# metaverse3d2022/Nerf-Cuda

Hardware: AMD Instinct MI355X
Metric: megasamples/s (march samples composited into a ray = the reference's per-ray sample count), Lego-like NeRF render @1920x1080 (higher is better)
Workload: dtype f16

## Files before the change

### nerf-cuda_amd/csrc/nrf_device.h

```cpp
#pragma once

#include <hip/hip_runtime.h>
#include <stdint.h>

#include "../../include/nerfhip.h"

namespace nrf {

typedef _Float16 half_t;
typedef _Float16 half2_t __attribute__((ext_vector_type(2)));
typedef _Float16 half4_t __attribute__((ext_vector_type(4)));
typedef _Float16 half8_t __attribute__((ext_vector_type(8)));
typedef float float2_t __attribute__((ext_vector_type(2)));
typedef float float4_t __attribute__((ext_vector_type(4)));

enum : uint32_t {
  LV_DENSE = 0,
  LV_HASH_POW2 = 1,
  LV_GENERIC = 2,
  LV_ADD_POW2 = 3
};

struct LevelParams {
  float scale;
// ... 610 lines not shown
  const uint32_t row = __umul24(gy, L.q_my_b) + L.q_off_b;
  const uint32_t slab = __umul24(gz, L.q_mz_b) + row;
  const uint32_t off0 = (gx << 4) + slab;
  const uint32_t off1 = off0 + L.q_mz_b;
  const __amdgpu_buffer_rsrc_t rsrc = __builtin_amdgcn_make_buffer_rsrc(const_cast<uint32_t*>(grid), 0, grid_bytes, 0x00020000);
  typedef uint32_t u32x4 __attribute__((ext_vector_type(4)));
  const u32x4 a = __builtin_amdgcn_raw_buffer_load_b128(rsrc, off0, 0, 0);
  const u32x4 b = __builtin_amdgcn_raw_buffer_load_b128(rsrc, off1, 0, 0);
  v[0] = a.x; v[1] = a.y; v[2] = a.z; v[3] = a.w;
  v[4] = b.x; v[5] = b.y; v[6] = b.z; v[7] = b.w;
}

__device__ __forceinline__ void level_gather_quad_far(const uint32_t* __restrict__ grid, const LevelParams L, float px, float py, float pz,
                                                      uint32_t (&v)[8], float (&frac)[3]) {
  float fx = px * L.scale; fx = fx + 0.5f;
  float fy = py * L.scale; fy = fy + 0.5f;
  float fz = pz * L.scale; fz = fz + 0.5f;
  uint32_t gx = (uint32_t)(int)fx, gy = (uint32_t)(int)fy, gz = (uint32_t)(int)fz;
  frac[0] = __builtin_amdgcn_fractf(fx);
  frac[1] = __builtin_amdgcn_fractf(fy);
  frac[2] = __builtin_amdgcn_fractf(fz);
  gx = gx < L.q_max ? gx : L.q_max;
  gy = gy < L.q_max ? gy : L.q_max;
  gz = gz < L.q_max ? gz : L.q_max;
  const uint32_t row = __umul24(gy, L.q_my_b) + L.q_off_b;
  const uint32_t cell = __umul24(gz, L.q_mz_b) + row + gx;
  const uint4* q = reinterpret_cast<const uint4*>(grid) + cell;
  const uint4 a = q[0];
  const uint4 b = q[L.q_mz_b];
  v[0] = a.x; v[1] = a.y; v[2] = a.z; v[3] = a.w;
  v[4] = b.x; v[5] = b.y; v[6] = b.z; v[7] = b.w;
}

template <bool FAST = false>
__device__ __forceinline__ uint32_t level_interp(const uint32_t (&v)[8], const float (&frac)[3]) {
  const float wx[2] = {1 - frac[0], frac[0]};
  const float wy[2] = {1 - frac[1], frac[1]};
  const float wz[2] = {1 - frac[2], frac[2]};
  if constexpr (FAST) {
    uint32_t a = 0u;
#pragma unroll
    for (int c = 0; c < 8; ++c) {
      const float w = (wx[c & 1] * wy[(c >> 1) & 1]) * wz[(c >> 2) & 1];
      asm("v_fma_mixlo_f16 %0, %1, %2, %0 op_sel_hi:[0,1,1]" : "+v"(a) : "v"(w), "v"(v[c]));
      asm("v_fma_mixhi_f16 %0, %1, %2, %0 op_sel:[0,1,1] op_sel_hi:[0,1,1]" : "+v"(a) : "v"(w), "v"(v[c]));
    }
    return a;
  }
  half2_t acc = {(half_t)0.0f, (half_t)0.0f};
#ifdef NRF_DIAG_DROP_INTERP_CVT
  float diag_acc_lo = 0.f, diag_acc_hi = 0.f;
#endif
#pragma unroll
  for (int c = 0; c < 8; ++c) {
    const float w = (wx[c & 1] * wy[(c >> 1) & 1]) * wz[(c >> 2) & 1];
#ifdef NRF_DIAG_DROP_INTERP_CVT
    {
      float lo, hi;
      const float neg_zero = -0.0f;
      asm("v_fma_mix_f32 %0, %1, %2, %3 op_sel_hi:[0,1,0]" : "=v"(lo) : "v"(w), "v"(v[c]), "v"(neg_zero));
      asm("v_fma_mix_f32 %0, %1, %2, %3 op_sel:[0,1,0] op_sel_hi:[0,1,0]" : "=v"(hi) : "v"(w), "v"(v[c]), "v"(neg_zero));
      diag_acc_lo += lo;
      diag_acc_hi += hi;
    }
#else
    acc = acc + weight_times_entry(w, v[c]);
// ... 201 lines not shown

__device__ __forceinline__ half8_t frag_load(const uint4* wl, int f, int lane) {
  const uint4 v = wl[f * 64 + lane];
  return __builtin_bit_cast(half8_t, v);
}

__device__ __forceinline__ half8_t pack_acc(float4_t lo, float4_t hi) {
#ifdef NRF_PROBE_NO_PACK
  typedef uint32_t u4 __attribute__((ext_vector_type(4)));
  return __builtin_bit_cast(half8_t, __builtin_bit_cast(u4, lo) ^ __builtin_bit_cast(u4, hi));
#endif
  half8_t r;
  r[0] = (half_t)lo[0]; r[1] = (half_t)lo[1]; r[2] = (half_t)lo[2]; r[3] = (half_t)lo[3];
  r[4] = (half_t)hi[0]; r[5] = (half_t)hi[1]; r[6] = (half_t)hi[2]; r[7] = (half_t)hi[3];
  const half8_t zero8 = {(half_t)0.f, (half_t)0.f, (half_t)0.f, (half_t)0.f, (half_t)0.f, (half_t)0.f, (half_t)0.f, (half_t)0.f};
  return __builtin_elementwise_max(r, zero8);
}

struct LdsFrags {
  const uint4* wl;
  int lane;
  __device__ __forceinline__ half8_t operator()(int f) const { return frag_load(wl, f >= FRAG_R0X ? f - FRAG_R0X + N_FRAGS : f, lane); }
};
struct LdsFragsPlain {
  const uint4* wl;
  int lane;
  __device__ __forceinline__ half8_t operator()(int f) const { return frag_load(wl, f, lane); }
};
template <int NT>
struct MlpOut {
  uint32_t rg[NT], bx[NT];
  half_t sigma;
};
template <int NT, int D0_BASE = FRAG_D0, typename Frags = LdsFrags, int RK = 1, int W = 64>
__device__ __forceinline__ void mlp_tiles(const Frags frag, const half8_t (&feat)[NT], const half4_t (&dirf)[NT], MlpOut<NT>& out,
                                          bool rgb_sigmoid = false, const half8_t (*dirx)[RK_WIDE - 1] = nullptr) {
  static_assert(NT == 1 || NT == 2 || NT == 4, "tiles per pass");
  using S = MlpShape<W>;
  constexpr int MT = S::MT, KS = S::KS;
  const float4_t zero = {0.f, 0.f, 0.f, 0.f};
  float4_t acc[NT][MT];
  half8_t hb[NT][KS];
  auto repack = [&]() {
#pragma unroll
    for (int n = 0; n < NT; ++n)
#pragma unroll
      for (int s = 0; s < KS; ++s) hb[n][s] = pack_acc(acc[n][2 * s], 2 * s + 1 < MT ? acc[n][2 * s + 1] : zero);
  };
#pragma unroll
  for (int m = 0; m < MT; ++m) {
    const half8_t a = frag(D0_BASE + m);
#pragma unroll
    for (int n = 0; n < NT; ++n) acc[n][m] = mfma16(a, feat[n], zero);
  }
  repack();
  float4_t dacc[NT];
#pragma unroll
  for (int n = 0; n < NT; ++n) dacc[n] = zero;
#pragma unroll
  for (int s = 0; s < KS; ++s) {
    const half8_t a = frag(S::D1 + s);
#pragma unroll
    for (int n = 0; n < NT; ++n) dacc[n] = mfma16(a, hb[n][s], dacc[n]);
  }
  half8_t rin[NT];
  uint32_t d01[NT];
#pragma unroll
  for (int n = 0; n < NT; ++n) {
    half8_t r;
    r[0] = (half_t)dacc[n][0];
    r[1] = (half_t)dacc[n][1];
    r[2] = (half_t)dacc[n][2];
// ... 185 lines not shown
```

### nerf-cuda_amd/csrc/nrf_launch.h

```cpp
#pragma once
#include <hip/hip_runtime.h>
#include <math.h>
#include <stdint.h>

namespace nrf {
enum : int { NET_HOT = 0, NET_GENERIC = 1, NET_WIDE = 2, NET_W16 = 3, NET_W32 = 4, NET_W128 = 5, NET_WIDE_SH = 6, NET_DEPTH = 7,
             NET_GRID2 = 8, NET_GRID4 = 9, NET_GRID8 = 10, NET_GRID1 = 11, NET_ACT = 12 };
__host__ __device__ constexpr int net_grid_f(int net) {
  return net == NET_GRID2 ? 2 : (net == NET_GRID4 ? 4 : (net == NET_GRID8 ? 8 : (net == NET_GRID1 ? 1 : 0)));
}
__host__ __device__ constexpr int net_width(int net) { return net == NET_W16 ? 16 : (net == NET_W32 ? 32 : (net == NET_W128 ? 128 : 64)); }

enum : uint32_t { GFORM_MIXED = 0, GFORM_DENSE = 1, GFORM_HASHED = 2, GFORM_QUAD = 3, GFORM_QUAD_FAR = 4 };
__host__ __device__ constexpr uint32_t gather_plan(uint32_t f0, uint32_t f1, uint32_t f2, uint32_t f3) {
  return 0x10000u | f0 | (f1 << 4) | (f2 << 8) | (f3 << 12);
}
__host__ __device__ constexpr uint32_t gather_form(uint32_t plan, int jl) { return (plan >> (4 * jl)) & 15u; }
constexpr uint32_t GATHER_RUNTIME = 0;
constexpr uint32_t GATHER_QQFH = gather_plan(GFORM_QUAD, GFORM_QUAD, GFORM_QUAD_FAR, GFORM_HASHED);
constexpr uint32_t GATHER_QQHH = gather_plan(GFORM_QUAD, GFORM_QUAD, GFORM_HASHED, GFORM_HASHED);
constexpr uint32_t GATHER_DMHH = gather_plan(GFORM_DENSE, GFORM_MIXED, GFORM_HASHED, GFORM_HASHED);
inline uint32_t gather_plan_of(int own, uint32_t n_levels, uint32_t uni_modes, uint32_t quad_mask, uint32_t quad_far) {
  if (own != NET_HOT || n_levels != 16) return GATHER_RUNTIME;
  uint32_t f[4];
  for (int jl = 0; jl < 4; ++jl)
    f[jl] = ((quad_mask >> (4 * jl)) & 1u) ? (((quad_far >> jl) & 1u) ? GFORM_QUAD_FAR : GFORM_QUAD) : ((uni_modes >> (2 * jl)) & 3u);
  const uint32_t plan = gather_plan(f[0], f[1], f[2], f[3]);
  return plan == GATHER_QQFH || plan == GATHER_QQHH || plan == GATHER_DMHH ? plan : GATHER_RUNTIME;
}

struct DevModel;
struct FrameParams;
struct ViewBatch;

constexpr int RENDER_QUEUE_BYTES = 8 * 4;
constexpr int WIDE_GENERIC_MARCH_WAVES = 8;
hipError_t launch_render(const DevModel& M, const FrameParams& P, const ViewBatch& VB, void* rgba, void* depth, void* counters,
                         hipStream_t st, bool first_launch, unsigned* plan = nullptr, unsigned plan_cap = 0);
constexpr unsigned PLAN_CAP = 60u * 1024u;
constexpr size_t PLAN_BYTES = (4 + 2 * (size_t)PLAN_CAP) * 4;
hipError_t launch_build_quads(const void* table, uint32_t res, uint32_t size, bool hashed, void* quads, hipStream_t st);
hipError_t launch_encode_grid(const DevModel& M, const void* pos01, uint32_t n, void* out, hipStream_t st, bool fast_interp = false);
hipError_t launch_encode_dir(const DevModel& M, const void* dir01, uint32_t n, void* out, hipStream_t st);
hipError_t launch_mlp_forward(const DevModel& M, const void* feat, const void* dirfeat, uint32_t n, void* out, uint32_t repeat,
                              hipStream_t st);
hipError_t launch_network(const DevModel& M, const void* xyz, const void* dir, uint32_t n, void* sigma, void* rgb, hipStream_t st);
hipError_t launch_density_positions(uint32_t H, float k, void* xyz, void* dir, hipStream_t st);
hipError_t launch_density_update(const void* sigma, uint32_t n, float decay, int n_iterations, void* grid, hipStream_t st);
hipError_t launch_generate_rays(const DevModel& M, const FrameParams& P, void* rays_o, void* rays_d, void* nears, void* fars,
                                hipStream_t st);
hipError_t launch_march(const DevModel& M, float dt_gamma, const void* rays_o, const void* rays_d, const void* rays_t,
                        const void* fars, uint32_t n, uint32_t n_step, void* xyzs, void* dirs, void* deltas, hipStream_t st,
                        uint32_t perturb = 0);
hipError_t launch_composite(const void* sigmas, const void* rgbs, const void* deltas, uint32_t n, uint32_t n_step, void* rays_t,
                            void* state, hipStream_t st);
hipError_t launch_untile(const void* gathered, int shard_count, int tiles_per_shard, int C, int W, int H, int n_views, void* out,
                         hipStream_t st);
hipError_t launch_untile_rgbd8_u8(const void* gathered, int shard_count, int tiles_per_shard, int W, int H, int n_views, void* rgb8,
                                  void* depth8, hipStream_t st);
hipError_t launch_quantize_rgbd8(const void* rgba, const void* depth, uint64_t n, void* out, hipStream_t st);
hipError_t launch_quantize(const void* rgba, const void* depth, int n, void* rgb8, void* depth8, hipStream_t st);
enum : int { MARCH_FORM_GENERIC = 0, MARCH_FORM_UNIT = 1, MARCH_FORM_POW2 = 2 };
inline int march_form(uint32_t H, uint32_t cascade, float bound) {
  const bool pow2_h = H != 0 && (H & (H - 1)) == 0;
  int eb = 0;
  if (pow2_h && cascade == 1 && bound >= 1.0f) return MARCH_FORM_UNIT;
  if (pow2_h && cascade > 1 && bound >= 1.0f && frexpf(bound, &eb) == 0.5f) return MARCH_FORM_POW2;
  return MARCH_FORM_GENERIC;
}
int render_persist_waves(int net, int form);
int render_persistent_lds_bytes(int net, int waves, uint32_t gen_wave_bytes);
void preload_kernels(bool all);
int render_lds_table_max_bytes();
int render_wide_lds_fixed_bytes();
int render_gen_lds_fixed_bytes(uint32_t gen_wave_bytes);
}
```

### nerf-cuda_amd/csrc/nrf_render.h

```cpp

#pragma once
#include <cstddef>
#include <cstdlib>

#include "nrf_device.h"
#include "nrf_generic.h"
#include "nrf_launch.h"

namespace nrf {

#ifndef NRF_SLOTS
#define NRF_SLOTS 64
#endif
constexpr int SLOTS = NRF_SLOTS;
struct WaveLds {
  union {
    float4 pos[SLOTS];
    float4 out[SLOTS];
  };
  float2 aux[SLOTS];
  uint32_t dirf[64][8];
};
static_assert(sizeof(WaveLds) == 2048 + 24 * SLOTS, "WaveLds layout");

// ... 138 lines not shown
          for (int e = 0; e < DW; ++e) fb[DW * jl + e] = o[e];
        }
      }
    }
  }
}

template <int RK, bool SHROWS>
__device__ __forceinline__ void gather_step(const DevModel& M, const LevelParams* lvs, int jl, int g, float px, float py, float pz,
                                            uint32_t (&v)[8], float (&fr)[3]) {
  const LevelParams L = lvs[4 * jl + g];
  const uint32_t uni = (M.uni_modes >> (2 * jl)) & 3u;
  if ((M.quad_mask >> (4 * jl)) & 1u) {
    constexpr bool FARQ = !(RK > 1 && !SHROWS);
    if (FARQ && ((M.quad_far >> jl) & 1u)) level_gather_quad_far(M.grid, L, px, py, pz, v, fr);
    else level_gather_quad(M.grid, M.grid_bytes, L, px, py, pz, v, fr);
  }
  else if (uni == 2u) level_gather<2>(M.grid, M.grid_bytes, L, px, py, pz, v, fr);
  else if (uni == 1u) level_gather<1>(M.grid, M.grid_bytes, L, px, py, pz, v, fr);
  else level_gather<0>(M.grid, M.grid_bytes, L, px, py, pz, v, fr);
}
template <uint32_t GP, int JL>
__device__ __forceinline__ void gather_step_static(const DevModel& M, const LevelParams* lvs, int g, float px, float py, float pz,
                                                   uint32_t (&v)[8], float (&fr)[3]) {
  constexpr uint32_t form = gather_form(GP, JL);
  static_assert(form <= GFORM_QUAD_FAR, "a static gather plan names one of the five step forms");
  const LevelParams L = lvs[4 * JL + g];
  if constexpr (form == GFORM_QUAD_FAR) level_gather_quad_far(M.grid, L, px, py, pz, v, fr);
  else if constexpr (form == GFORM_QUAD) level_gather_quad(M.grid, M.grid_bytes, L, px, py, pz, v, fr);
  else if constexpr (form == GFORM_HASHED) level_gather<2>(M.grid, M.grid_bytes, L, px, py, pz, v, fr);
  else if constexpr (form == GFORM_DENSE) level_gather<1>(M.grid, M.grid_bytes, L, px, py, pz, v, fr);
  else level_gather<0>(M.grid, M.grid_bytes, L, px, py, pz, v, fr);
}
__device__ __forceinline__ void sample_pos01(const DevModel& M, const float4 p, float& px, float& py, float& pz) {
  if (M.pos_w_pow2) {
    px = __builtin_fmaf(M.pos_w, p.x, 0.5f);
    py = __builtin_fmaf(M.pos_w, p.y, 0.5f);
    pz = __builtin_fmaf(M.pos_w, p.z, 0.5f);
  } else {
    px = M.pos_w * p.x; px = px + 0.5f;
    py = M.pos_w * p.y; py = py + 0.5f;
    pz = M.pos_w * p.z; pz = pz + 0.5f;
  }
}

template <int NT, int RK = 1, bool FAST = false, int WD = 64, bool SHROWS = false, int DEPTH = 0, int GF = 0, uint32_t GP = GATHER_RUNTIME>
__device__ __forceinline__ void network_from_lds(const DevModel& M, const uint4* wl, const LevelParams* lvs, WaveLds* W,
                                                 const float* rayd, int S, int base, int lane, float density_scale,
                                                 const half_t* rows = nullptr) {
  const int g = lane >> 4, c = lane & 15;
  half8_t feat[NT];
  half4_t dirf[NT];
  half8_t dirx[NT][RK_WIDE - 1];
#pragma unroll
  for (int n = 0; n < NT; ++n) {
    const int slot = base + 16 * n + c;
    uint32_t fb[4] = {0u, 0u, 0u, 0u};
    uint2 db = make_uint2(0u, 0u);
    if (slot < S) {
      const float4 p = W->pos[slot];
      float px, py, pz;
      sample_pos01(M, p, px, py, pz);
      if constexpr (GF != 0) {
        grid_features<GF>(M, lvs, px, py, pz, g, fb);
      } else {
      uint32_t gv[4][8];
      float gf[4][3];
      if constexpr (GP != GATHER_RUNTIME) {
        static_assert(RK == 1, "static gather plans exist for the hot instance only");
        gather_step_static<GP, 0>(M, lvs, g, px, py, pz, gv[0], gf[0]);
        gather_step_static<GP, 1>(M, lvs, g, px, py, pz, gv[1], gf[1]);
        gather_step_static<GP, 2>(M, lvs, g, px, py, pz, gv[2], gf[2]);
        gather_step_static<GP, 3>(M, lvs, g, px, py, pz, gv[3], gf[3]);
      } else {
#pragma unroll
      for (int jl = 0; jl < 4; ++jl) gather_step<RK, SHROWS>(M, lvs, jl, g, px, py, pz, gv[jl], gf[jl]);
      }
#pragma unroll
      for (int jl = 0; jl < 4; ++jl) fb[jl] = level_interp<FAST>(gv[jl], gf[jl]);
      }
      const int ray = __builtin_bit_cast(int, p.w);
      db = *reinterpret_cast<const uint2*>(&W->dirf[ray][2 * g]);
      if constexpr (RK > 1 && SHROWS) {
        const half8_t z8 = {(half_t)0.f, (half_t)0.f, (half_t)0.f, (half_t)0.f, (half_t)0.f, (half_t)0.f, (half_t)0.f, (half_t)0.f};
#pragma unroll
        for (int s = 1; s < RK; ++s) {
          const uint32_t e0 = 32u * s - 16u + 8u * (uint32_t)g;
          dirx[n][s - 1] = e0 < M.dir_w ? *reinterpret_cast<const half8_t*>(rows + (size_t)ray * SH_ROW_HALVES + e0) : z8;
        }
      } else if constexpr (RK > 1) {
        const float dx = rayd[3 * ray], dy = rayd[3 * ray + 1], dz = rayd[3 * ray + 2];
#pragma unroll
        for (int s = 1; s < RK; ++s) dirx[n][s - 1] = dir_entries8(M.n_frequencies, 32u * s - 16u + 8u * (uint32_t)g, dx, dy, dz);
      }
    } else if constexpr (RK > 1) {
      const half8_t z8 = {(half_t)0.f, (half_t)0.f, (half_t)0.f, (half_t)0.f, (half_t)0.f, (half_t)0.f, (half_t)0.f, (half_t)0.f};
#pragma unroll
      for (int s = 1; s < RK; ++s) dirx[n][s - 1] = z8;
    }
    const uint4 fv = make_uint4(fb[0], fb[1], fb[2], fb[3]);
    feat[n] = __builtin_bit_cast(half8_t, fv);
    dirf[n] = __builtin_bit_cast(half4_t, db);
  }
  MlpOut<NT> o;
  if constexpr (DEPTH == 2) mlp_tiles_depth<NT, LdsFragsPlain, true>(LdsFragsPlain{wl, lane}, feat, dirf, o, M.rgb_output_activation == NRF_ACT_SIGMOID, M.depth_xd,
                                                                     M.depth_xr, M.density_activation, M.rgb_activation);
  else if constexpr (DEPTH == 1) mlp_tiles_depth<NT>(LdsFragsPlain{wl, lane}, feat, dirf, o, M.rgb_output_activation == NRF_ACT_SIGMOID, M.depth_xd, M.depth_xr);
  else if constexpr (WD == 64) mlp_tiles<NT, FRAG_D0, LdsFrags, RK>(LdsFrags{wl, lane}, feat, dirf, o, M.rgb_output_activation == NRF_ACT_SIGMOID, dirx);
  else mlp_tiles<NT, 0, LdsFragsPlain, 1, WD>(LdsFragsPlain{wl, lane}, feat, dirf, o, M.rgb_output_activation == NRF_ACT_SIGMOID);
  if (g == 0) {
#pragma unroll
    for (int n = 0; n < NT; ++n) {
      const int slot = base + 16 * n + c;
      const half2_t rg = bits_h2(o.rg[n]), bx = bits_h2(o.bx[n]);
      if (slot < S) *reinterpret_cast<float3*>(&W->out[slot]) = make_float3((float)rg.x, (float)rg.y, (float)bx.x);
    }
  }
  if (g < NT) {
    const int slot = base + 16 * g + c;
    float sigma = (float)o.sigma;
    if (density_scale != 1.0f) sigma = density_scale * sigma;
    if (slot < S) W->out[slot].w = sigma;
  }
}

constexpr int NT_MAX = 2;

template <bool DENSITY_ONLY>
__device__ __forceinline__ void gen_network_from_lds(const DevModel& M, const GenModel& G, const LevelParams* lvs, WaveLds* W,
                                                     const GenLds& Lw, int S, int base, int lane, float density_scale) {
  const int g = lane >> 4, c = lane & 15;
  float p01[GEN_TILES][3];
  bool valid[GEN_TILES];
  int ray[GEN_TILES];
#pragma unroll
  for (int n = 0; n < GEN_TILES; ++n) {
    const int slot = base + 16 * n + c;
    valid[n] = slot < S;
    ray[n] = 0;
    p01[n][0] = p01[n][1] = p01[n][2] = 0.5f;
// ... 1 lines not shown
      const float4 p = W->pos[slot];
      float px = M.pos_w * p.x; px = px + 0.5f;
      float py = M.pos_w * p.y; py = py + 0.5f;
      float pz = M.pos_w * p.z; pz = pz + 0.5f;
      p01[n][0] = px; p01[n][1] = py; p01[n][2] = pz;
      ray[n] = __builtin_bit_cast(int, p.w) & 63;
    }
  }
  gen_encode_rows(M, G, lvs, Lw, lane, p01, valid);
  if constexpr (!DENSITY_ONLY) {
    const int slot = base + lane;
    if (lane < GEN_SAMPLES && slot < S) {
      const int r = __builtin_bit_cast(int, W->pos[slot].w) & 63;
      gen_encode_dir(M, G, Lw.rayd[3 * r], Lw.rayd[3 * r + 1], Lw.rayd[3 * r + 2], Lw.dir + (size_t)lane * G.dir_stride);
    }
#pragma unroll
    for (int n = 0; n < GEN_TILES; ++n) ray[n] = 16 * n + c;
  }
  gen_wave_sync();
  float4_t o[GEN_TILES];
  gen_mlps<DENSITY_ONLY>(M, G, Lw, lane, ray, o);
  if (g == 0) {
#pragma unroll
    for (int n = 0; n < GEN_TILES; ++n) {
      const int slot = base + 16 * n + c;
      float sigma = o[n][3];
      if (density_scale != 1.0f) sigma = density_scale * sigma;
      if (slot < S) W->out[slot] = make_float4(o[n][0], o[n][1], o[n][2], sigma);
    }
  }
  gen_wave_sync();
}

template <int NET, bool FAST = false, uint32_t GP = GATHER_RUNTIME>
__device__ __forceinline__ void network_dispatch(const DevModel& M, const uint4* wl, const LevelParams* lvs, WaveLds* W,
                                                 const GenLds& Lw, int S, int lane, float density_scale) {
  constexpr int RK = (NET == NET_WIDE || NET == NET_WIDE_SH) ? RK_WIDE : 1;
  constexpr bool SHR = NET == NET_WIDE_SH;
  if constexpr (NET == NET_GENERIC) {
    const GenModel& G = *M.gen;
    for (int base = 0; base < S; base += GEN_SAMPLES)
      gen_network_from_lds<false>(M, G, lvs, W, Lw, S, base, lane, density_scale);
  } else {
    constexpr int WD = net_width(NET);
    constexpr int NTM = WD == 128 ? 1 : NT_MAX;
    for (int base = 0; base < S; base += 16 * NTM) {
      const int ntile = (S - base + 15) >> 4;
      constexpr int DP = NET == NET_DEPTH ? 1 : (NET == NET_ACT ? 2 : 0);
      constexpr int GF = net_grid_f(NET);
      if (ntile <= 1 || NTM == 1) network_from_lds<1, RK, FAST, WD, SHR, DP, GF, GP>(M, wl, lvs, W, Lw.rayd, S, base, lane, density_scale, Lw.dir);
      else network_from_lds<NTM, RK, FAST, WD, SHR, DP, GF, GP>(M, wl, lvs, W, Lw.rayd, S, base, lane, density_scale, Lw.dir);
    }
  }
}

struct LdsMap {
  uint4* wl;
  LevelParams* lvs;
  WaveLds* W;
  GenLds gen;
  unsigned char* tables;
};
template <int NET>
__device__ __forceinline__ LdsMap lds_map(unsigned char* smem, const DevModel& M, int wave, int n_waves) {
  LdsMap m;
  if constexpr (NET == NET_GENERIC) {
    const GenModel& G = *M.gen;
    m.lvs = reinterpret_cast<LevelParams*>(smem);
    unsigned char* waves = smem + LDS_LEVEL_BYTES;
    m.W = reinterpret_cast<WaveLds*>(waves) + wave;
    unsigned char* dir = waves + n_waves * (int)sizeof(WaveLds);
    unsigned char* act = dir + n_waves * gen_dir_bytes(G);
    m.wl = reinterpret_cast<uint4*>(act);
    m.gen.dens = reinterpret_cast<half_t*>(&m.W->dirf[0][0]);
    m.gen.rayd = reinterpret_cast<float*>(&m.W->dirf[32][0]);
    m.gen.dir = reinterpret_cast<half_t*>(dir + wave * gen_dir_bytes(G));
    m.gen.X = reinterpret_cast<half_t*>(act + wave * gen_act_bytes(G));
    m.gen.Y = m.gen.X + GEN_SAMPLES * G.act_stride;
    m.gen.wfrag = M.wfrag;
    m.tables = act + n_waves * gen_act_bytes(G);
  } else {
    constexpr int WF = net_wfrag_bytes(NET);
    m.wl = reinterpret_cast<uint4*>(smem);
    m.lvs = reinterpret_cast<LevelParams*>(smem + WF);
// ... 293 lines not shown
                                                     rdy, rdz, sx, sy, sz, far_m, t_skip, budget, t, x, y, z, dt);
        found = r == MARCH_FOUND;
        marching = found;
        ended = ended || r == MARCH_EXHAUSTED;
      }
#ifdef NRF_PHASE_TIMING
      {
        int used = budget_before - budget;
        n_lane_trips += (unsigned)used;
        for (int o = 32; o; o >>= 1) used = max(used, __shfl_xor(used, o));
        n_wave_iters += (unsigned)used;
      }
#endif
      const unsigned long long fm = __ballot(found);
      if (found) {
        const int slot = S + (int)__builtin_amdgcn_mbcnt_hi((unsigned)(fm >> 32), __builtin_amdgcn_mbcnt_lo((unsigned)fm, 0u));
        const float tn = t + dt;
        const float delta = tn - last_t;
        tc = tc + delta;
        t = tc;
        W->pos[slot] = make_float4(x, y, z, __builtin_bit_cast(float, lane));
        W->aux[slot] = make_float2(dt, tc);
        slots |= (unsigned long long)slot << (8 * k);
        cnt++;
        if (n_ray_samples + cnt >= P.max_steps) { marching = false; ended = true; }
        else if (cnt >= cap) marching = false;
      }
      S += __popcll(fm);
    }
    wave_sync();
    NRF_STAMP(t1);

    if (S > 0) {
      network_dispatch<NET, FAST, GP>(M, wl, lvs, W, lm.gen, S, lane, P.density_scale);
      wave_sync();
    }
    NRF_STAMP(t2);

    if (alive) {
      bool terminated = false;
      for (int k = 0; k < 8; ++k) {
        if (k >= cnt) break;
        const int slot = (int)((slots >> (8 * k)) & 0xffull);
        const float4 so = W->out[slot];
        const float2 dtc = W->aux[slot];
        const float alpha = 1.0f - __expf(-so.w * dtc.x);
        const float T = 1 - ws;
        const float wgt = alpha * T;
        ws += wgt;
        dep += wgt * dtc.y;
        cr += wgt * so.x;
        cg += wgt * so.y;
        cb += wgt * so.z;
        n_comp++;
        if (T <= 9.99999974737875e-05f) { terminated = true; break; }
      }
      n_ray_samples += cnt;
      alive = !(terminated || ended);
    }
    wave_sync();
    NRF_STAMP(t3);
    NRF_ACC(c_march, t0, t1);
    NRF_ACC(c_net, t1, t2);
    NRF_ACC(c_comp, t2, t3);
    n_samples += (unsigned)S;
    n_rounds++;
    n_tile_slots += (unsigned)((S + 15) & ~15);
// ... 303 lines not shown
          uint32_t GP = GATHER_RUNTIME, bool FAST = false>
__global__ __launch_bounds__(64 * WAVES, 1) void render_persistent_kernel(const DevModel M0, const FrameParams P0, const ViewBatch VB0,
                                                                              float4* __restrict__ rgba0, float* __restrict__ depth0,
                                                                              unsigned long long* __restrict__ counters,
                                                                              unsigned* __restrict__ queue) {
  extern __shared__ __attribute__((aligned(16))) unsigned char smem[];
  const int wave = __builtin_amdgcn_readfirstlane((int)(threadIdx.x >> 6));
  const int lane = lane_id();
  typedef const PersistArgs __attribute__((address_space(4))) * KArgPtr;
  KArgPtr ka = (KArgPtr)__builtin_amdgcn_kernarg_segment_ptr();
  const DevModel& M = M0;
  const FrameParams& P = P0;
  const ViewBatch& VB = VB0;
  constexpr int PERSIST_WAVES = WAVES;
  constexpr bool GEN = NET == NET_GENERIC;
  constexpr int OUT8 = U8 ? 1 : 0;
  LdsMap lm = lds_map<NET>(smem, M, wave, PERSIST_WAVES);
  uint32_t* coarse_lds = reinterpret_cast<uint32_t*>(lm.tables);
  float* ctab_lds = reinterpret_cast<float*>(coarse_lds + M.lds_coarse_words);
  uint32_t* dil_lds = reinterpret_cast<uint32_t*>(ctab_lds + M.lds_ctab_floats);
  int* q_lds = reinterpret_cast<int*>(dil_lds + M.lds_dilated_words);
  unsigned* sched = reinterpret_cast<unsigned*>(q_lds + MAX_VIEWS + 1);
  HelpLds* hl = reinterpret_cast<HelpLds*>(sched + 1);
  static_assert(WAVES <= 16, "HelpLds::mail / idle_mask hold 16 waves");
  if constexpr (!GEN) stage_fragments<NET>(M, lm.wl);
  if constexpr (GEN && WLDS) {
    uint4* w_lds = reinterpret_cast<uint4*>(smem + ((reinterpret_cast<unsigned char*>(hl + 1) + LDS_CLOCK_BYTES - smem + 15) & ~(size_t)15));
    for (uint32_t i = threadIdx.x; i < M.gen_frag_bytes / 16u; i += blockDim.x) w_lds[i] = M.wfrag[i];
    lm.gen.wfrag = w_lds;
  }
  for (uint32_t i = threadIdx.x; i < M.lds_coarse_words; i += blockDim.x) coarse_lds[i] = M.occ_coarse[i];
  for (uint32_t i = threadIdx.x; i < M.lds_ctab_floats; i += blockDim.x) ctab_lds[i] = M.cell_bound[i];
  for (uint32_t i = threadIdx.x; i < M.lds_dilated_words; i += blockDim.x) dil_lds[i] = M.occ_dilated[i];
  if (threadIdx.x < 16) lm.lvs[threadIdx.x] = M.lv[threadIdx.x];
  if (threadIdx.x <= MAX_VIEWS) {
    const int v = (int)threadIdx.x;
    q_lds[v] = v < VB.n_views ? VB.v[v].q_begin : VB.q_total;
  }
  if (threadIdx.x == 0) *sched = (0xfffffeu << 5) | 4u;
  if (threadIdx.x == 0) {
    hl->idle_mask = 0u;
    hl->busy = PERSIST_WAVES;
  }
  if (threadIdx.x < 16) hl->mail[threadIdx.x] = 0u;
  __syncthreads();
#ifndef NRF_PHASE_TIMING
  unsigned* clk_lds = reinterpret_cast<unsigned*>(hl + 1);
  if (wave == 0) {
    unsigned long long t0, r0;
    asm volatile("s_memtime %0\n\ts_memrealtime %1\n\ts_waitcnt lgkmcnt(0)" : "=s"(t0), "=s"(r0)::"memory");
    if (lane == 0) {
      clk_lds[0] = (unsigned)t0;
      clk_lds[1] = (unsigned)(t0 >> 32);
      clk_lds[2] = (unsigned)r0;
      clk_lds[3] = (unsigned)(r0 >> 32);
    }
  }
#endif

  const MarchConst mc = march_const(M, P.dt_gamma);
  TileStats ts;
  const unsigned n_cls = (unsigned)VB0.n_classes, cls_cols = (unsigned)VB0.class_cols, n_units = (unsigned)VB0.q_total;
  const unsigned cls0 = (__builtin_amdgcn_s_getreg(20 | (0 << 6) | (3 << 11)) & 15u) % n_cls;
  constexpr unsigned POS_DONE = 0xffffffu;
  NRF_STAMP(t_loop_begin);
#ifdef NRF_PHASE_TIMING
  unsigned long long c_sched = 0;
// ... 405 lines not shown
```

### nerf-cuda_amd/csrc/nrf_api.hip

```cpp

#include <hip/hip_runtime.h>

#include <chrono>
#include <cmath>
#include <cstdio>
#include <cstdlib>
#include <cstring>
#include <limits>
#include <mutex>
#include <string>
#include <vector>

#include "nrf_device.h"
#include "nrf_generic.h"
#include "nrf_launch.h"

using namespace nrf;

namespace {

thread_local std::string g_err;
int fail(int code, const std::string& msg) {
  g_err = msg;
  return code;
// ... 1708 lines not shown
  if (!c || !c->model_loaded) return -1;
  if (c->rays_persistent) return 16;
  const int st = (int)c->dm.stage;
  return st == NET_GENERIC ? 1 : st == NET_WIDE ? 2 : 0;
}

extern "C" int nrf_debug_ray_valid(const float o[3], const float d[3]) {
  if (!o || !d) return 0;
  return ray_valid(o, d) ? 1 : 0;
}

extern "C" int nrf_debug_plan(const nrf_model_desc* d, int allow_own, uint64_t budget_mb, uint32_t out[6]) {
  if (!d || !d->params || !out) return fail(NRF_E_INVALID, "null argument");
  const ModelPlan p = plan_model(*d, allow_own != 0, budget_mb, 4);
  if (p.rc) return p.rc;
  const int waves = render_persist_waves(p.own, march_form(d->density_grid_size, d->cascade, d->bound));
  const uint32_t v[6] = {(uint32_t)p.own, (uint32_t)p.stage, p.quad_mask, p.quad_far, (uint32_t)waves,
                         (uint32_t)render_persistent_lds_bytes(p.own, waves, p.gen_wave_bytes)};
  std::memcpy(out, v, sizeof(v));
  return NRF_OK;
}

extern "C" int nrf_debug_gather_plan(const nrf_model_desc* d, int allow_own, uint64_t budget_mb, uint32_t out[5]) {
  if (!d || !d->params || !out) return fail(NRF_E_INVALID, "null argument");
  const char* e = std::getenv("NRF_GATHER_PLAN");
  const ModelPlan p = plan_model(*d, allow_own != 0, budget_mb ? budget_mb : (uint64_t)QUAD_BUDGET_MB_DEFAULT, 4, !(e && std::atoi(e) == 0));
  if (p.rc) return p.rc;
  out[0] = p.gather_plan;
  for (int jl = 0; jl < 4; ++jl)
    out[1 + jl] = ((p.quad_mask >> (4 * jl)) & 1u) ? (((p.quad_far >> jl) & 1u) ? GFORM_QUAD_FAR : GFORM_QUAD) : ((p.uni_modes >> (2 * jl)) & 3u);
  return NRF_OK;
}

extern "C" int nrf_debug_wave_times(nrf_context* c, unsigned long long* out, int n_waves) {
  if (!c || !out || n_waves < 1 || n_waves > 4096) return fail(NRF_E_INVALID, "bad argument");
  HIP_TRY(hipEventSynchronize(c->ev1));
  HIP_TRY(hipMemcpy(out, call_slot(c, c->call_index) + COUNTER_BYTES + 128, (size_t)n_waves * 16, hipMemcpyDeviceToHost));
  return NRF_OK;
}

int nrf_render_async(nrf_context* c, const float cam[4], const float pose[16], nrf_frame* out) {
  if (!c) return fail(NRF_E_INVALID, "null context");
  return nrf_render(c, cam, pose, (void*)c->stream, out);
}

int nrf_sync(nrf_context* c) {
  if (!c) return fail(NRF_E_INVALID, "null context");
  int rc = set_device(c);
  if (rc) return rc;
  HIP_TRY(hipStreamSynchronize(c->stream));
  if (c->last_stream && c->last_stream != c->stream) HIP_TRY(hipStreamSynchronize(c->last_stream));
  return NRF_OK;
}

int nrf_bind_output(nrf_context* c, void* rgba, void* depth) {
  if (!c) return fail(NRF_E_INVALID, "null context");
  if ((rgba == nullptr) != (depth == nullptr)) return fail(NRF_E_INVALID, "bind both planes or neither");
  c->bound_rgba = rgba;
  c->bound_depth = depth;
  c->bound_rgbd8 = nullptr;
  c->bound_rgb8 = c->bound_depth8 = nullptr;
  return NRF_OK;
}

int nrf_bind_output_rgbd8(nrf_context* c, void* rgbd8) {
  if (!c) return fail(NRF_E_INVALID, "null context");
// ... 272 lines not shown
```

Before: 15570.

## Software-pipeline static-plan hash gathers across tiles with branchless slot masking

For the static gather-plan hot path, feature gathering moves into a dedicated routine. It issues the long-latency gather level of the second tile early, alongside the first tile's gathers, and pins the order with sched_barriers. Out-of-range slots are clamped and their results masked instead of branched around, so loads can be issued uniformly. This aims to hide global-memory gather latency behind other work, at the cost of more live registers, which may reduce occupancy.

New measurement: 15430. No clear change (-0.9%).

```diff
diff --git a/nerf-cuda_amd/csrc/nrf_device.h b/nerf-cuda_amd/csrc/nrf_device.h
--- a/nerf-cuda_amd/csrc/nrf_device.h
+++ b/nerf-cuda_amd/csrc/nrf_device.h
@@ -666,6 +666,15 @@
   v[4] = b.x; v[5] = b.y; v[6] = b.z; v[7] = b.w;
 }
 
+__device__ __forceinline__ void level_fractions(const LevelParams L, float px, float py, float pz, float (&frac)[3]) {
+  float fx = px * L.scale; fx = fx + 0.5f;
+  float fy = py * L.scale; fy = fy + 0.5f;
+  float fz = pz * L.scale; fz = fz + 0.5f;
+  frac[0] = __builtin_amdgcn_fractf(fx);
+  frac[1] = __builtin_amdgcn_fractf(fy);
+  frac[2] = __builtin_amdgcn_fractf(fz);
+}
+
 template <bool FAST = false>
 __device__ __forceinline__ uint32_t level_interp(const uint32_t (&v)[8], const float (&frac)[3]) {
   const float wx[2] = {1 - frac[0], frac[0]};
diff --git a/nerf-cuda_amd/csrc/nrf_launch.h b/nerf-cuda_amd/csrc/nrf_launch.h
--- a/nerf-cuda_amd/csrc/nrf_launch.h
+++ b/nerf-cuda_amd/csrc/nrf_launch.h
@@ -20,6 +20,7 @@
 constexpr uint32_t GATHER_QQFH = gather_plan(GFORM_QUAD, GFORM_QUAD, GFORM_QUAD_FAR, GFORM_HASHED);
 constexpr uint32_t GATHER_QQHH = gather_plan(GFORM_QUAD, GFORM_QUAD, GFORM_HASHED, GFORM_HASHED);
 constexpr uint32_t GATHER_DMHH = gather_plan(GFORM_DENSE, GFORM_MIXED, GFORM_HASHED, GFORM_HASHED);
+__host__ __device__ constexpr int gather_long_step(uint32_t plan) { return gather_form(plan, 2) == GFORM_QUAD_FAR ? 2 : 3; }
 inline uint32_t gather_plan_of(int own, uint32_t n_levels, uint32_t uni_modes, uint32_t quad_mask, uint32_t quad_far) {
   if (own != NET_HOT || n_levels != 16) return GATHER_RUNTIME;
   uint32_t f[4];
diff --git a/nerf-cuda_amd/csrc/nrf_render.h b/nerf-cuda_amd/csrc/nrf_render.h
--- a/nerf-cuda_amd/csrc/nrf_render.h
+++ b/nerf-cuda_amd/csrc/nrf_render.h
@@ -206,6 +206,73 @@
   }
 }
 
+__device__ __forceinline__ void sample_pos01_flat(const DevModel& M, const float4 p, float& px, float& py, float& pz) {
+  px = M.pos_w * p.x; px = px + 0.5f;
+  py = M.pos_w * p.y; py = py + 0.5f;
+  pz = M.pos_w * p.z; pz = pz + 0.5f;
+}
+
+template <int NT, uint32_t GP, bool FAST>
+__device__ __forceinline__ void plan_features(const DevModel& M, const LevelParams* lvs, const WaveLds* W, int S, int base, int g, int c,
+                                              half8_t (&feat)[NT], half4_t (&dirf)[NT]) {
+  static_assert(NT == 1 || NT == 2, "a pass is one or two tiles");
+  constexpr int LS = gather_long_step(GP);
+  constexpr int A = LS > 0 ? 0 : 1, B = LS > 1 ? 1 : 2, C = LS > 2 ? 2 : 3;
+  uint32_t gv[NT][4][8], fb[NT][4];
+  float gf[NT][4][3];
+  const int slot0 = base + c < S ? base + c : S - 1;
+  float px, py, pz;
+  const float4 p0 = W->pos[slot0];
+  sample_pos01_flat(M, p0, px, py, pz);
+  __builtin_amdgcn_sched_barrier(0);
+  gather_step_static<GP, A>(M, lvs, g, px, py, pz, gv[0][A], gf[0][A]);
+  gather_step_static<GP, B>(M, lvs, g, px, py, pz, gv[0][B], gf[0][B]);
+  gather_step_static<GP, C>(M, lvs, g, px, py, pz, gv[0][C], gf[0][C]);
+  __builtin_amdgcn_sched_barrier(0);
+  gather_step_static<GP, LS>(M, lvs, g, px, py, pz, gv[0][LS], gf[0][LS]);
+  __builtin_amdgcn_sched_barrier(0);
+  int slot1 = base + 16 + c < S ? base + 16 + c : S - 1;
+  if constexpr (NT == 2) {
+    float qx, qy, qz, fr[3];
+    sample_pos01_flat(M, W->pos[slot1], qx, qy, qz);
+    gather_step_static<GP, LS>(M, lvs, g, qx, qy, qz, gv[1][LS], fr);
+    asm volatile("" : "+v"(slot1));
+    __builtin_amdgcn_sched_barrier(0);
+  }
+  fb[0][A] = level_interp<FAST>(gv[0][A], gf[0][A]);
+  fb[0][B] = level_interp<FAST>(gv[0][B], gf[0][B]);
+  fb[0][C] = level_interp<FAST>(gv[0][C], gf[0][C]);
+  fb[0][LS] = level_interp<FAST>(gv[0][LS], gf[0][LS]);
+  int ray[NT];
+  ray[0] = __builtin_bit_cast(int, p0.w);
+  if constexpr (NT == 2) {
+    __builtin_amdgcn_sched_barrier(0);
+    const float4 p1 = W->pos[slot1];
+    sample_pos01_flat(M, p1, px, py, pz);
+    ray[1] = __builtin_bit_cast(int, p1.w);
+    gather_step_static<GP, A>(M, lvs, g, px, py, pz, gv[1][A], gf[1][A]);
+    gather_step_static<GP, B>(M, lvs, g, px, py, pz, gv[1][B], gf[1][B]);
+    gather_step_static<GP, C>(M, lvs, g, px, py, pz, gv[1][C], gf[1][C]);
+    __builtin_amdgcn_sched_barrier(0);
+    level_fractions(lvs[4 * LS + g], px, py, pz, gf[1][LS]);
+    fb[1][LS] = level_interp<FAST>(gv[1][LS], gf[1][LS]);
+    fb[1][A] = level_interp<FAST>(gv[1][A], gf[1][A]);
+    fb[1][B] = level_interp<FAST>(gv[1][B], gf[1][B]);
+    fb[1][C] = level_interp<FAST>(gv[1][C], gf[1][C]);
+  }
+  __builtin_amdgcn_sched_barrier(0);
+#pragma unroll
+  for (int n = 0; n < NT; ++n) {
+    uint32_t keep = base + 16 * n + c < S ? 0xffffffffu : 0u;
+    asm volatile("" : "+v"(keep));
+    const uint2 db = *reinterpret_cast<const uint2*>(&W->dirf[ray[n]][2 * g]);
+    const uint4 fv = make_uint4(fb[n][0] & keep, fb[n][1] & keep, fb[n][2] & keep, fb[n][3] & keep);
+    const uint2 dv = make_uint2(db.x & keep, db.y & keep);
+    feat[n] = __builtin_bit_cast(half8_t, fv);
+    dirf[n] = __builtin_bit_cast(half4_t, dv);
+  }
+}
+
 template <int NT, int RK = 1, bool FAST = false, int WD = 64, bool SHROWS = false, int DEPTH = 0, int GF = 0, uint32_t GP = GATHER_RUNTIME>
 __device__ __forceinline__ void network_from_lds(const DevModel& M, const uint4* wl, const LevelParams* lvs, WaveLds* W,
                                                  const float* rayd, int S, int base, int lane, float density_scale,
@@ -214,6 +281,10 @@
   half8_t feat[NT];
   half4_t dirf[NT];
   half8_t dirx[NT][RK_WIDE - 1];
+  if constexpr (GP != GATHER_RUNTIME) {
+    static_assert(RK == 1 && GF == 0, "static gather plans exist for the hot instance only");
+    plan_features<NT, GP, FAST>(M, lvs, W, S, base, g, c, feat, dirf);
+  } else {
 #pragma unroll
   for (int n = 0; n < NT; ++n) {
     const int slot = base + 16 * n + c;
@@ -228,16 +299,8 @@
       } else {
       uint32_t gv[4][8];
       float gf[4][3];
-      if constexpr (GP != GATHER_RUNTIME) {
-        static_assert(RK == 1, "static gather plans exist for the hot instance only");
-        gather_step_static<GP, 0>(M, lvs, g, px, py, pz, gv[0], gf[0]);
-        gather_step_static<GP, 1>(M, lvs, g, px, py, pz, gv[1], gf[1]);
-        gather_step_static<GP, 2>(M, lvs, g, px, py, pz, gv[2], gf[2]);
-        gather_step_static<GP, 3>(M, lvs, g, px, py, pz, gv[3], gf[3]);
-      } else {
 #pragma unroll
       for (int jl = 0; jl < 4; ++jl) gather_step<RK, SHROWS>(M, lvs, jl, g, px, py, pz, gv[jl], gf[jl]);
-      }
 #pragma unroll
       for (int jl = 0; jl < 4; ++jl) fb[jl] = level_interp<FAST>(gv[jl], gf[jl]);
       }
@@ -263,6 +326,7 @@
     const uint4 fv = make_uint4(fb[0], fb[1], fb[2], fb[3]);
     feat[n] = __builtin_bit_cast(half8_t, fv);
     dirf[n] = __builtin_bit_cast(half4_t, db);
+  }
   }
   MlpOut<NT> o;
   if constexpr (DEPTH == 2) mlp_tiles_depth<NT, LdsFragsPlain, true>(LdsFragsPlain{wl, lane}, feat, dirf, o, M.rgb_output_activation == NRF_ACT_SIGMOID, M.depth_xd,
```

## Pack plan-specific level params in LDS and prefetch MLP weight fragments

Applied to the files above, without the earlier changes.

For static gather plans, the persistent kernel stages each hash-grid level's parameters in LDS as a compact two-uint4 block tailored to that level's gather form. It loads all four per-thread level params up front and separates the per-level gathers with scheduling barriers. It also adds a software prefetch of MLP weight fragments from LDS to a configurable depth, overlapping the first fragment loads with the last level's interpolation. The aim is to cut LDS latency and scalar/vector load stalls in the gather-then-MLP hot path, at the cost of extra registers (possible occupancy loss) and tighter scheduling constraints.

Result: faster. 15530 before, 15750 after (median of 6 runs) (+1.4%).

```diff
diff --git a/nerf-cuda_amd/csrc/nrf_api.hip b/nerf-cuda_amd/csrc/nrf_api.hip
--- a/nerf-cuda_amd/csrc/nrf_api.hip
+++ b/nerf-cuda_amd/csrc/nrf_api.hip
@@ -1764,6 +1764,15 @@
   return NRF_OK;
 }
 
+extern "C" int nrf_debug_lds_schedule(uint32_t plan, int form, uint32_t out[2]) {
+  if (!out) return fail(NRF_E_INVALID, "null argument");
+  if (plan != GATHER_RUNTIME && plan != GATHER_QQFH && plan != GATHER_QQHH && plan != GATHER_DMHH) return fail(NRF_E_INVALID, "not a gather plan");
+  if (form != MARCH_FORM_GENERIC && form != MARCH_FORM_UNIT && form != MARCH_FORM_POW2) return fail(NRF_E_INVALID, "not a march form");
+  out[0] = plan_levels(plan) ? 1u : 0u;
+  out[1] = (uint32_t)plan_frag_depth(plan, form);
+  return NRF_OK;
+}
+
 extern "C" int nrf_debug_wave_times(nrf_context* c, unsigned long long* out, int n_waves) {
   if (!c || !out || n_waves < 1 || n_waves > 4096) return fail(NRF_E_INVALID, "bad argument");
   HIP_TRY(hipEventSynchronize(c->ev1));
diff --git a/nerf-cuda_amd/csrc/nrf_device.h b/nerf-cuda_amd/csrc/nrf_device.h
--- a/nerf-cuda_amd/csrc/nrf_device.h
+++ b/nerf-cuda_amd/csrc/nrf_device.h
@@ -933,12 +933,32 @@
   uint32_t rg[NT], bx[NT];
   half_t sigma;
 };
-template <int NT, int D0_BASE = FRAG_D0, typename Frags = LdsFrags, int RK = 1, int W = 64>
-__device__ __forceinline__ void mlp_tiles(const Frags frag, const half8_t (&feat)[NT], const half4_t (&dirf)[NT], MlpOut<NT>& out,
-                                          bool rgb_sigmoid = false, const half8_t (*dirx)[RK_WIDE - 1] = nullptr) {
+template <int NT, int D0_BASE = FRAG_D0, typename Frags = LdsFrags, int RK = 1, int W = 64, int PF = 0>
+__device__ __forceinline__ void mlp_tiles(const Frags frag_lds, const half8_t (&feat)[NT], const half4_t (&dirf)[NT], MlpOut<NT>& out,
+                                          bool rgb_sigmoid = false, const half8_t (*dirx)[RK_WIDE - 1] = nullptr,
+                                          const half8_t* pre = nullptr) {
   static_assert(NT == 1 || NT == 2 || NT == 4, "tiles per pass");
+  static_assert(PF == 0 || RK == 1, "the fragment prefetch covers the fragments 0 .. S::N - 1");
   using S = MlpShape<W>;
   constexpr int MT = S::MT, KS = S::KS;
+  half8_t wq[PF > 0 ? PF : 1];
+  int wn = 0;
+  if constexpr (PF > 0) {
+#pragma unroll
+    for (int i = 0; i < PF; ++i) wq[i] = pre[i];
+  }
+  auto frag = [&](int f) -> half8_t {
+    if constexpr (PF > 0) {
+      const half8_t a = wq[wn % PF];
+      const int ahead = wn + PF;
+      if (ahead < S::N) wq[wn % PF] = frag_lds(ahead < MT ? D0_BASE + ahead : ahead);
+      ++wn;
+      __builtin_amdgcn_sched_barrier(0x676);
+      return a;
+    } else {
+      return frag_lds(f);
+    }
+  };
   const float4_t zero = {0.f, 0.f, 0.f, 0.f};
   float4_t acc[NT][MT];
   half8_t hb[NT][KS];
diff --git a/nerf-cuda_amd/csrc/nrf_launch.h b/nerf-cuda_amd/csrc/nrf_launch.h
--- a/nerf-cuda_amd/csrc/nrf_launch.h
+++ b/nerf-cuda_amd/csrc/nrf_launch.h
@@ -68,6 +68,19 @@
   if (pow2_h && cascade > 1 && bound >= 1.0f && frexpf(bound, &eb) == 0.5f) return MARCH_FORM_POW2;
   return MARCH_FORM_GENERIC;
 }
+#ifndef NRF_LDS_PARAMS
+#define NRF_LDS_PARAMS 1
+#endif
+#ifndef NRF_LDS_FRAG_DEPTH
+#define NRF_LDS_FRAG_DEPTH 2
+#endif
+#ifndef NRF_LDS_FRAG_DEPTH_GENERIC
+#define NRF_LDS_FRAG_DEPTH_GENERIC (NRF_LDS_FRAG_DEPTH > 1 ? 1 : NRF_LDS_FRAG_DEPTH)
+#endif
+__host__ __device__ constexpr bool plan_levels(uint32_t gp) { return gp != GATHER_RUNTIME && NRF_LDS_PARAMS != 0; }
+__host__ __device__ constexpr int plan_frag_depth(uint32_t gp, int march) {
+  return gp == GATHER_RUNTIME ? 0 : (march == MARCH_FORM_GENERIC ? NRF_LDS_FRAG_DEPTH_GENERIC : NRF_LDS_FRAG_DEPTH);
+}
 int render_persist_waves(int net, int form);
 int render_persistent_lds_bytes(int net, int waves, uint32_t gen_wave_bytes);
 void preload_kernels(bool all);
diff --git a/nerf-cuda_amd/csrc/nrf_render.h b/nerf-cuda_amd/csrc/nrf_render.h
--- a/nerf-cuda_amd/csrc/nrf_render.h
+++ b/nerf-cuda_amd/csrc/nrf_render.h
@@ -194,6 +194,51 @@
   else if constexpr (form == GFORM_DENSE) level_gather<1>(M.grid, M.grid_bytes, L, px, py, pz, v, fr);
   else level_gather<0>(M.grid, M.grid_bytes, L, px, py, pz, v, fr);
 }
+static_assert(MARCH_GENERIC == MARCH_FORM_GENERIC && MARCH_UNIT == MARCH_FORM_UNIT && MARCH_POW2 == MARCH_FORM_POW2, "plan_frag_depth's march form");
+static_assert(LDS_LEVEL_BYTES >= 16 * 32, "the staged plan levels live in the level table's region");
+template <uint32_t GP>
+__device__ __forceinline__ void stage_plan_level(LevelParams* lvs, uint32_t l, const LevelParams L) {
+  const uint32_t form = gather_form(GP, (int)(l >> 2));
+  const uint32_t sc = __builtin_bit_cast(uint32_t, L.scale);
+  uint4 a, b = make_uint4(L.mask_b, L.mode, 0u, 0u);
+  if (form == GFORM_QUAD || form == GFORM_QUAD_FAR) a = make_uint4(sc, L.q_off_b, L.q_my_b, L.q_mz_b);
+  else if (form == GFORM_HASHED) a = make_uint4(sc, L.off_b, L.mask_b, 0u);
+  else a = make_uint4(sc, L.off_b, L.my_b, L.mz_b);
+  uint4* blk = reinterpret_cast<uint4*>(lvs) + 2 * l;
+  blk[0] = a;
+  blk[1] = b;
+}
+template <uint32_t GP, int JL>
+__device__ __forceinline__ LevelParams plan_level(const LevelParams* lvs, int g) {
+  constexpr uint32_t form = gather_form(GP, JL);
+  const uint4* blk = reinterpret_cast<const uint4*>(lvs) + 2 * (4 * JL + g);
+  const uint4 a = blk[0];
+  LevelParams L = {};
+  L.scale = __builtin_bit_cast(float, a.x);
+  if constexpr (form == GFORM_QUAD || form == GFORM_QUAD_FAR) {
+    L.q_off_b = a.y; L.q_my_b = a.z; L.q_mz_b = a.w;
+    if constexpr (form == GFORM_QUAD_FAR) L.q_max = a.z - 1u;
+  } else if constexpr (form == GFORM_HASHED) {
+    L.off_b = a.y; L.mask_b = a.z;
+  } else {
+    L.off_b = a.y; L.my_b = a.z; L.mz_b = a.w;
+    if constexpr (form == GFORM_MIXED) {
+      const uint4 b = blk[1];
+      L.mask_b = b.x; L.mode = b.y;
+    }
+  }
+  return L;
+}
+template <uint32_t GP, int JL>
+__device__ __forceinline__ void gather_step_level(const DevModel& M, const LevelParams& L, float px, float py, float pz,
+                                                  uint32_t (&v)[8], float (&fr)[3]) {
+  constexpr uint32_t form = gather_form(GP, JL);
+  if constexpr (form == GFORM_QUAD_FAR) level_gather_quad_far(M.grid, L, px, py, pz, v, fr);
+  else if constexpr (form == GFORM_QUAD) level_gather_quad(M.grid, M.grid_bytes, L, px, py, pz, v, fr);
+  else if constexpr (form == GFORM_HASHED) level_gather<2>(M.grid, M.grid_bytes, L, px, py, pz, v, fr);
+  else if constexpr (form == GFORM_DENSE) level_gather<1>(M.grid, M.grid_bytes, L, px, py, pz, v, fr);
+  else level_gather<0>(M.grid, M.grid_bytes, L, px, py, pz, v, fr);
+}
 __device__ __forceinline__ void sample_pos01(const DevModel& M, const float4 p, float& px, float& py, float& pz) {
   if (M.pos_w_pow2) {
     px = __builtin_fmaf(M.pos_w, p.x, 0.5f);
@@ -206,7 +251,8 @@
   }
 }
 
-template <int NT, int RK = 1, bool FAST = false, int WD = 64, bool SHROWS = false, int DEPTH = 0, int GF = 0, uint32_t GP = GATHER_RUNTIME>
+template <int NT, int RK = 1, bool FAST = false, int WD = 64, bool SHROWS = false, int DEPTH = 0, int GF = 0, uint32_t GP = GATHER_RUNTIME,
+          int PF = 0>
 __device__ __forceinline__ void network_from_lds(const DevModel& M, const uint4* wl, const LevelParams* lvs, WaveLds* W,
                                                  const float* rayd, int S, int base, int lane, float density_scale,
                                                  const half_t* rows = nullptr) {
@@ -214,13 +260,24 @@
   half8_t feat[NT];
   half4_t dirf[NT];
   half8_t dirx[NT][RK_WIDE - 1];
+  half8_t wpre[PF > 0 ? PF : 1];
 #pragma unroll
   for (int n = 0; n < NT; ++n) {
     const int slot = base + 16 * n + c;
     uint32_t fb[4] = {0u, 0u, 0u, 0u};
     uint2 db = make_uint2(0u, 0u);
+    uint32_t lastv[8];
+    float lastf[3];
     if (slot < S) {
       const float4 p = W->pos[slot];
+      LevelParams PL[4];
+      if constexpr (plan_levels(GP) && GF == 0) {
+        PL[0] = plan_level<GP, 0>(lvs, g);
+        PL[1] = plan_level<GP, 1>(lvs, g);
+        PL[2] = plan_level<GP, 2>(lvs, g);
+        PL[3] = plan_level<GP, 3>(lvs, g);
+        __builtin_amdgcn_sched_barrier(0);
+      }
       float px, py, pz;
       sample_pos01(M, p, px, py, pz);
       if constexpr (GF != 0) {
@@ -228,7 +285,16 @@
       } else {
       uint32_t gv[4][8];
       float gf[4][3];
-      if constexpr (GP != GATHER_RUNTIME) {
+      if constexpr (plan_levels(GP)) {
+        static_assert(RK == 1, "static gather plans exist for the hot instance only");
+        gather_step_level<GP, 0>(M, PL[0], px, py, pz, gv[0], gf[0]);
+        __builtin_amdgcn_sched_barrier(0x78f);
+        gather_step_level<GP, 1>(M, PL[1], px, py, pz, gv[1], gf[1]);
+        __builtin_amdgcn_sched_barrier(0x78f);
+        gather_step_level<GP, 2>(M, PL[2], px, py, pz, gv[2], gf[2]);
+        __builtin_amdgcn_sched_barrier(0x78f);
+        gather_step_level<GP, 3>(M, PL[3], px, py, pz, gv[3], gf[3]);
+      } else if constexpr (GP != GATHER_RUNTIME) {
         static_assert(RK == 1, "static gather plans exist for the hot instance only");
         gather_step_static<GP, 0>(M, lvs, g, px, py, pz, gv[0], gf[0]);
         gather_step_static<GP, 1>(M, lvs, g, px, py, pz, gv[1], gf[1]);
@@ -239,7 +305,15 @@
       for (int jl = 0; jl < 4; ++jl) gather_step<RK, SHROWS>(M, lvs, jl, g, px, py, pz, gv[jl], gf[jl]);
       }
 #pragma unroll
-      for (int jl = 0; jl < 4; ++jl) fb[jl] = level_interp<FAST>(gv[jl], gf[jl]);
+      for (int jl = 0; jl < 4; ++jl) {
+        if (PF > 0 && n == NT - 1 && jl == 3) {
+#pragma unroll
+          for (int k = 0; k < 8; ++k) lastv[k] = gv[3][k];
+          lastf[0] = gf[3][0]; lastf[1] = gf[3][1]; lastf[2] = gf[3][2];
+        } else {
+          fb[jl] = level_interp<FAST>(gv[jl], gf[jl]);
+        }
+      }
       }
       const int ray = __builtin_bit_cast(int, p.w);
       db = *reinterpret_cast<const uint2*>(&W->dirf[ray][2 * g]);
@@ -260,6 +334,15 @@
 #pragma unroll
       for (int s = 1; s < RK; ++s) dirx[n][s - 1] = z8;
     }
+    if constexpr (PF > 0) {
+      if (n == NT - 1) {
+        const LdsFrags frag{wl, lane};
+#pragma unroll
+        for (int f = 0; f < PF; ++f) wpre[f] = frag(FRAG_D0 + f);
+        __builtin_amdgcn_sched_barrier(0);
+        if (slot < S) fb[3] = level_interp<FAST>(lastv, lastf);
+      }
+    }
     const uint4 fv = make_uint4(fb[0], fb[1], fb[2], fb[3]);
     feat[n] = __builtin_bit_cast(half8_t, fv);
     dirf[n] = __builtin_bit_cast(half4_t, db);
@@ -268,6 +351,10 @@
   if constexpr (DEPTH == 2) mlp_tiles_depth<NT, LdsFragsPlain, true>(LdsFragsPlain{wl, lane}, feat, dirf, o, M.rgb_output_activation == NRF_ACT_SIGMOID, M.depth_xd,
                                                                      M.depth_xr, M.density_activation, M.rgb_activation);
   else if constexpr (DEPTH == 1) mlp_tiles_depth<NT>(LdsFragsPlain{wl, lane}, feat, dirf, o, M.rgb_output_activation == NRF_ACT_SIGMOID, M.depth_xd, M.depth_xr);
+  else if constexpr (WD == 64 && PF > 0) {
+    static_assert(RK == 1, "the fragment prefetch exists for the hot instance only");
+    mlp_tiles<NT, FRAG_D0, LdsFrags, 1, 64, PF>(LdsFrags{wl, lane}, feat, dirf, o, M.rgb_output_activation == NRF_ACT_SIGMOID, nullptr, wpre);
+  }
   else if constexpr (WD == 64) mlp_tiles<NT, FRAG_D0, LdsFrags, RK>(LdsFrags{wl, lane}, feat, dirf, o, M.rgb_output_activation == NRF_ACT_SIGMOID, dirx);
   else mlp_tiles<NT, 0, LdsFragsPlain, 1, WD>(LdsFragsPlain{wl, lane}, feat, dirf, o, M.rgb_output_activation == NRF_ACT_SIGMOID);
   if (g == 0) {
@@ -335,7 +422,7 @@
   gen_wave_sync();
 }
 
-template <int NET, bool FAST = false, uint32_t GP = GATHER_RUNTIME>
+template <int NET, bool FAST = false, uint32_t GP = GATHER_RUNTIME, int PF = 0>
 __device__ __forceinline__ void network_dispatch(const DevModel& M, const uint4* wl, const LevelParams* lvs, WaveLds* W,
                                                  const GenLds& Lw, int S, int lane, float density_scale) {
   constexpr int RK = (NET == NET_WIDE || NET == NET_WIDE_SH) ? RK_WIDE : 1;
@@ -351,8 +438,8 @@
       const int ntile = (S - base + 15) >> 4;
       constexpr int DP = NET == NET_DEPTH ? 1 : (NET == NET_ACT ? 2 : 0);
       constexpr int GF = net_grid_f(NET);
-      if (ntile <= 1 || NTM == 1) network_from_lds<1, RK, FAST, WD, SHR, DP, GF, GP>(M, wl, lvs, W, Lw.rayd, S, base, lane, density_scale, Lw.dir);
-      else network_from_lds<NTM, RK, FAST, WD, SHR, DP, GF, GP>(M, wl, lvs, W, Lw.rayd, S, base, lane, density_scale, Lw.dir);
+      if (ntile <= 1 || NTM == 1) network_from_lds<1, RK, FAST, WD, SHR, DP, GF, GP, PF>(M, wl, lvs, W, Lw.rayd, S, base, lane, density_scale, Lw.dir);
+      else network_from_lds<NTM, RK, FAST, WD, SHR, DP, GF, GP, PF>(M, wl, lvs, W, Lw.rayd, S, base, lane, density_scale, Lw.dir);
     }
   }
 }
@@ -712,7 +799,7 @@
     NRF_STAMP(t1);
 
     if (S > 0) {
-      network_dispatch<NET, FAST, GP>(M, wl, lvs, W, lm.gen, S, lane, P.density_scale);
+      network_dispatch<NET, FAST, GP, plan_frag_depth(GP, MARCH)>(M, wl, lvs, W, lm.gen, S, lane, P.density_scale);
       wave_sync();
     }
     NRF_STAMP(t2);
@@ -1082,7 +1169,11 @@
   for (uint32_t i = threadIdx.x; i < M.lds_coarse_words; i += blockDim.x) coarse_lds[i] = M.occ_coarse[i];
   for (uint32_t i = threadIdx.x; i < M.lds_ctab_floats; i += blockDim.x) ctab_lds[i] = M.cell_bound[i];
   for (uint32_t i = threadIdx.x; i < M.lds_dilated_words; i += blockDim.x) dil_lds[i] = M.occ_dilated[i];
-  if (threadIdx.x < 16) lm.lvs[threadIdx.x] = M.lv[threadIdx.x];
+  if constexpr (plan_levels(GP)) {
+    if (threadIdx.x < 16) stage_plan_level<GP>(lm.lvs, threadIdx.x, M.lv[threadIdx.x]);
+  } else {
+    if (threadIdx.x < 16) lm.lvs[threadIdx.x] = M.lv[threadIdx.x];
+  }
   if (threadIdx.x <= MAX_VIEWS) {
     const int v = (int)threadIdx.x;
     q_lds[v] = v < VB.n_views ? VB.v[v].q_begin : VB.q_total;
```
